# uthree/ALiVE-VC

Hardware: AMD Instinct MI355X
Metric: VC frames/sec + RTF @24kHz, 1M-vec library; 1/2/4/8 MI355X (higher is better)
Workload: dtype decoder fp16 GEMMs / fp32 acc; encoders 22-bit fp16 split; kNN exact fp32 top-k via fp6 MFMA candidates (certified); f32 MFMA small convs; f64 phase scan

## Files before the change

### alive-vc_amd/csrc/knn.hip

```cpp
#include "common.h"

namespace {

constexpr int D = ALIVE_DIM;
constexpr int KP = ALIVE_KPRIME;
constexpr int TILE = 128;
constexpr int MAX_SPLIT = 64;

__device__ __forceinline__ float wave_sum(float v) {
#pragma unroll
    for (int o = 32; o > 0; o >>= 1) v += __shfl_xor(v, o);
    return v;
}

struct NormDiv {
    float n, y;
};
__device__ __forceinline__ NormDiv norm_div(float n) {
    float y = __builtin_amdgcn_rcpf(n);
    const float e = fmaf(-n, y, 1.0f);
    y = fmaf(e, y, y);
    return NormDiv{n, y};
}
__device__ __forceinline__ float div_by(float x, const NormDiv& d) {
// ... 88 lines not shown
                                                                 const float* __restrict__ norms, int64_t M,
                                                                 unsigned* __restrict__ bound) {
    const int lane = threadIdx.x & 63;
    const int64_t m = (int64_t)blockIdx.x * 4 + (threadIdx.x >> 6);
    if (m >= M) return;
    const float nn = norms[m];
    float ss = 0.0f;
    for (int d = lane; d < D; d += 64) {
        const float q = rows[(size_t)m * D + d] / nn;
        const float b = __uint_as_float((unsigned)lib[(size_t)m * D + d] << 16);
        const float e = q - b;
        ss = fmaf(e, e, ss);
    }
    ss = wave_sum(ss);
    if (lane == 0) atomicMax(bound, __float_as_uint(sqrtf(ss) * 1.0001f));
}

constexpr float F8_SCALE = 256.0f;
constexpr float F6_SCALE = 32.0f;
__device__ __forceinline__ unsigned fp6_e2m3(float y) {
    const unsigned sgn = (__float_as_uint(y) >> 31) << 5;
    const float a = fminf(fabsf(y), 7.5f);
    unsigned code;
    if (a < 1.0f) {
        code = (unsigned)__builtin_rintf(a * 8.0f);
    } else {
        unsigned b = __float_as_uint(a);
        b += 0x7FFFFu + ((b >> 20) & 1u);
        code = (b >> 20) - (126u << 3);
        code = code < 31u ? code : 31u;
    }
    return sgn | code;
}
__global__ __launch_bounds__(256) void to_fp6_kernel(const unsigned short* __restrict__ in, int64_t n32, int64_t n_valid, u32x4* __restrict__ out,
                                                     unsigned char* __restrict__ clip = nullptr) {
    const int64_t i = (int64_t)blockIdx.x * 256 + threadIdx.x;
    if (i >= n32) return;
    if (i >= n_valid) {
        out[2 * i] = u32x4{0u, 0u, 0u, 0u};
        out[2 * i + 1] = u32x4{0u, 0u, 0u, 0u};
        return;
    }
    unsigned long long acc = 0;
    int nb = 0, wi = 0;
    unsigned wd[6];
    bool clipped = false;
#pragma unroll
    for (int j = 0; j < 32; ++j) {
        const float v = __uint_as_float((unsigned)in[i * 32 + j] << 16) * F6_SCALE;
        clipped = clipped || fabsf(v) > 7.75f;
        acc |= (unsigned long long)fp6_e2m3(v) << nb;
        nb += 6;
        if (nb >= 32) { wd[wi++] = (unsigned)acc; acc >>= 32; nb -= 32; }
    }
    out[2 * i] = u32x4{wd[0], wd[1], wd[2], wd[3]};
    out[2 * i + 1] = u32x4{wd[4], wd[5], 0u, 0u};
    if (clip != nullptr && clipped) clip[i / (D / 32)] = 1;
}
__device__ __forceinline__ unsigned char to_fp8(float v) {
    return (unsigned char)(__builtin_amdgcn_cvt_pk_fp8_f32(v * F8_SCALE, 0.0f, 0, false) & 0xff);
}
__device__ __forceinline__ unsigned to_fp8x4(float a, float b, float c, float d) {
    int w = __builtin_amdgcn_cvt_pk_fp8_f32(a * F8_SCALE, b * F8_SCALE, 0, false);
    w = __builtin_amdgcn_cvt_pk_fp8_f32(c * F8_SCALE, d * F8_SCALE, w, true);
    return (unsigned)w;
}

__global__ __launch_bounds__(256) void lib_to_fp8_kernel(const unsigned short* __restrict__ lib, int64_t n8, uint2* __restrict__ out) {
    const int64_t i = (int64_t)blockIdx.x * 256 + threadIdx.x;
    if (i >= n8) return;
    const u32x4 v = ((const u32x4*)lib)[i];
    float f[8];
#pragma unroll
    for (int j = 0; j < 4; ++j) {
        f[2 * j] = __uint_as_float(v[j] << 16);
        f[2 * j + 1] = __uint_as_float(v[j] & 0xffff0000u);
    }
    out[i] = make_uint2(to_fp8x4(f[0], f[1], f[2], f[3]), to_fp8x4(f[4], f[5], f[6], f[7]));
}

__global__ __launch_bounds__(256) void src_to_fp8_kernel(const unsigned short* __restrict__ s_bf16, int64_t n8, uint2* __restrict__ out) {
    const int64_t i = (int64_t)blockIdx.x * 256 + threadIdx.x;
    if (i >= n8) return;
    const u32x4 v = ((const u32x4*)s_bf16)[i];
    float f[8];
#pragma unroll
    for (int j = 0; j < 4; ++j) {
        f[2 * j] = __uint_as_float(v[j] << 16);
        f[2 * j + 1] = __uint_as_float(v[j] & 0xffff0000u);
    }
// ... 2173 lines not shown
    bool clipped = false;
#pragma unroll
    for (int h = 0; h < 2; ++h) {
#pragma unroll
        for (int j = 0; j < 32; ++j) {
            v[j] = live ? yb[(size_t)(32 * (cg + 8 * h) + j) * T] * inv : 0.0f;
            sy = fmaf(v[j], v[j], sy);
            v[j] *= F6_SCALE;
        }
        u32x4 o[2];
        clipped = fp6_slot(v, o) || clipped;
        if (f < Tt_pad) {
            u32x4* dst = (u32x4*)(out + (size_t)f * SUB_K + 32 * (cg + 8 * h));
            dst[0] = o[0];
            dst[1] = o[1];
        }
    }
    const float gy = live ? yb[(size_t)SUB_K * T] * inv : 0.0f;
    if (cg == 0) sy = fmaf(gy, gy, sy);
    ssq[cg][fl] = sy;
    clp[cg][fl] = clipped ? 1 : 0;
    __syncthreads();
    if (cg == 0 && f < Tt_pad) {
        float s2 = 0.0f;
        int cl = 0;
#pragma unroll
        for (int k = 0; k < 8; ++k) { s2 += ssq[k][fl]; cl |= clp[k][fl]; }
        const bool out_of_span = q > 0.0f && 1.0f - s2 > SUB_RES2;
        const bool bad = live && (cl != 0 || out_of_span);
        g[f] = gy;
        flag[f] = bad ? 1 : 0;
        if (bad) atomicAdd(stats + ST_SUB_FLAG, 1);
        if (live && cl != 0) atomicAdd(stats + ST_SUB_CLIP, 1);
    }
}
__global__ __launch_bounds__(256) void sub_select_kernel(const unsigned char* __restrict__ flag, unsigned char* __restrict__ clip6,
                                                         int64_t n, int* __restrict__ stats) {
    const bool sub = stats[ST_SUB_FLAG] <= RESEARCH_MIN;
    const int64_t i = (int64_t)blockIdx.x * 256 + threadIdx.x;
    if (sub && i < n && flag[i] != 0) clip6[i] = 1;
    if (i == 0) {
        stats[ST_SUB_FORM] = sub ? 1 : 2;
        stats[ST_SUB_GATE] = stats[ST_MODE] != 0 ? 0 : (sub ? 1 : 2);
    }
}

__global__ void stats_init_kernel(int* __restrict__ stats, int tier, int hist_tag = 0) {
    if (threadIdx.x < ST_HIST_TAG)
        stats[threadIdx.x] = threadIdx.x == ST_TIER ? tier
                           : threadIdx.x == ST_RESEARCH_MIN ? RESEARCH_MIN : threadIdx.x == ST_COLLECT_MIN ? COLLECT_MIN : 0;
    if (threadIdx.x == ST_HIST_TAG) {
        const bool valid = hist_tag != 0 && stats[ST_HIST_TAG] == hist_tag;
        const int streak = valid ? stats[ST_HIST_STREAK] : 0, calls = valid ? stats[ST_HIST_CALLS] : 0;
        const bool skip = streak >= PROBE_STREAK && (calls % PROBE_EVERY) != 0;
        stats[ST_HIST_TAG] = hist_tag;
        stats[ST_HIST_STREAK] = streak;
        stats[ST_HIST_CALLS] = calls + 1;
        stats[ST_PROBE_GATE] = skip ? 0 : 1;
        stats[ST_PROBE_SKIPPED] = skip ? 1 : 0;
    }
}
__global__ void probe_history_kernel(int* __restrict__ stats, int64_t Tt) {
    const bool clean = stats[ST_MODE] == 0 && (int64_t)stats[ST_FLAG8] * 20 <= Tt &&
                       (stats[ST_PROBE_GATE] == 0 || (int64_t)stats[ST_PROBE_FAIL] * 4 <= (int64_t)stats[ST_PROBE_N]);
    stats[ST_HIST_STREAK] = clean ? stats[ST_HIST_STREAK] + 1 : 0;
}
// ... 505 lines not shown
    if (g_ev_start) (void)hipEventRecord(g_ev_start, s);
    knn_scan_kernel<true><<<blocks, 64 * SCAN_WAVES, 0, s>>>(s_f32, rows_f32, norms, M, (int)Tt, k, pv, pi);
    if (g_ev_stop) (void)hipEventRecord(g_ev_stop, s);
    if (k <= 4) knn_scan_merge_kernel<true><<<(unsigned)Tt, 256, 0, s>>>(pv, pi, blocks * SCAN_WAVES, k, idx_base, out_val, out_idx);
    else knn_scan_merge_kernel<false><<<(unsigned)Tt, 256, 0, s>>>(pv, pi, blocks * SCAN_WAVES, k, idx_base, out_val, out_idx);
    ALIVE_CHECK_LAUNCH("alive_knn_search(scan)");
    return ALIVE_OK;
}

static void knn_exact_launch(const SearchWs& w, const float* rows_f32, const float* norms, int64_t M, int64_t Tt, int64_t idx_base,
                             int k, const int* list, const int* cnt, float* out_val, int32_t* out_idx, hipStream_t s,
                             int max_count = 0x7fffffff) {
#define ALIVE_EXACT(G_)                                                                                                        \
    {                                                                                                                          \
        knn_exact_kernel<G_><<<EX_BLOCKS, 256, 0, s>>>(w.s_f32, rows_f32, norms, M, Tt, k, list, cnt, w.pv, w.pi, max_count);   \
        knn_exact_merge_kernel<G_><<<1024, 256, 0, s>>>(w.pv, w.pi, Tt, k, idx_base, list, cnt, out_val, out_idx, max_count);  \
    }
    switch (exact_group(k)) {
        case 16: ALIVE_EXACT(16) break;
        case 8: ALIVE_EXACT(8) break;
        case 4: ALIVE_EXACT(4) break;
        case 2: ALIVE_EXACT(2) break;
        default: ALIVE_EXACT(1) break;
    }
#undef ALIVE_EXACT
}

static void src_prep_launch(const SearchWs& w, const float* src, int T, int64_t Tt, hipStream_t s) {
    float* dq = w.det_q != nullptr ? w.dq : nullptr;
    if (Tt <= 512) src_prep_small_kernel<<<(unsigned)w.p16.Tt_pad, 256, 0, s>>>(src, T, Tt, w.s_f32, w.s_bf16, dq, w.sub_nrm);
    else src_prep_kernel<<<(unsigned)(w.p16.Tt_pad / 64), 256, 0, s>>>(src, T, Tt, w.p16.Tt_pad, w.s_f32, w.s_bf16, dq, w.sub_nrm);
}

static int check_search_args(const char* what, const void* a, const void* b, int N, int T, int k, int64_t M) {
    ALIVE_CHECK_ARG(a && b, "%s: null pointer", what);
    ALIVE_CHECK_ARG(N > 0 && T > 0, "%s: empty source", what);
    ALIVE_CHECK_ARG(k >= 1 && k <= ALIVE_MAX_K, "%s: k=%d outside [1,%d]", what, k, ALIVE_MAX_K);
    ALIVE_CHECK_ARG(M >= k, "%s: library shard has %lld vectors, fewer than k=%d", what, (long long)M, k);
    ALIVE_CHECK_ARG((int64_t)N * T < ((int64_t)1 << 31) - FT6, "%s: %lld frames in one call", what, (long long)N * T);
    return ALIVE_OK;
}

static int lds_optin(const char* what) {
    static LdsOptIn optin8, optin6, optin16, optin_split, optin_sub;
    hipError_t e = optin8.ensure({(const void*)knn_score8_kernel, (const void*)knn_probe8_kernel}, SCORE8_LDS);
    if (e == hipSuccess) e = optin6.ensure({(const void*)knn_score6_kernel, (const void*)knn_probe6_kernel}, SCORE6_LDS);
    if (e == hipSuccess) e = optin16.ensure({(const void*)knn_score_kernel<false>, (const void*)knn_score_kernel<true>}, SCORE_LDS);
    if (e == hipSuccess) e = optin_split.ensure({(const void*)knn_collect_split_kernel}, SPLIT_LDS);
    if (e == hipSuccess) e = optin_sub.ensure({(const void*)knn_sub6_kernel}, SUB6_LDS);
    if (e != hipSuccess) {
        alive_set_error("%s: cannot reserve %d B of LDS: %s", what, SCORE_LDS, hipGetErrorString(e));
        return ALIVE_ERR_LAUNCH;
    }
    return ALIVE_OK;
}

extern "C" size_t alive_library_fp8_bytes(int64_t M) { return (size_t)alive_library_padded_rows(M) * D; }

extern "C" int alive_library_pack_fp8(const void* lib_bf16, int64_t M, void* lib_f8, void* stream) {
    ALIVE_CHECK_ARG(lib_bf16 && lib_f8 && M >= 1, "alive_library_pack_fp8: bad args");
    const int64_t n8 = alive_library_padded_rows(M) * D / 8;
    lib_to_fp8_kernel<<<(unsigned)((n8 + 255) / 256), 256, 0, (hipStream_t)stream>>>((const unsigned short*)lib_bf16, n8, (uint2*)lib_f8);
    ALIVE_CHECK_LAUNCH("alive_library_pack_fp8");
    return ALIVE_OK;
}

// ... 166 lines not shown
}

extern "C" int alive_knn_search_timed(const float* src, int N, int T, const void* lib_bf16, const float* rows_f32,
                                      const float* norms, int64_t M, int64_t idx_base, int k, float* out_val, int32_t* out_idx,
                                      void* ws, void* stream, void* ev_start, void* ev_stop) {
    return knn_search_impl(src, N, T, lib_bf16, rows_f32, norms, M, idx_base, k, out_val, out_idx, ws, stream,
                           (hipEvent_t)ev_start, (hipEvent_t)ev_stop);
}

static int knn_search_fp8_impl(const float* src, int N, int T, const void* lib_f8, const void* lib_bf16, const float* rows_f32,
                               const float* norms, int64_t M, int64_t idx_base, int k, float* out_val, int32_t* out_idx,
                               void* ws, void* stream, hipEvent_t g_ev_start, hipEvent_t g_ev_stop, int fmt = 0,
                               const float* y_rot = nullptr, float rot_c0 = 0.0f, const float* y_sub = nullptr,
                               const void* lib_sub = nullptr, const float* rho = nullptr) {
    ALIVE_CHECK_ARG(src && lib_f8 && lib_bf16 && rows_f32 && norms && out_val && out_idx && ws, "alive_knn_search_fp8: null pointer");
    if (int rc = check_search_args("alive_knn_search_fp8", src, ws, N, T, k, M)) return rc;
    const int64_t Tt = (int64_t)N * T;
    if (k > KH)
        return knn_search_impl(src, N, T, lib_bf16, rows_f32, norms, M, idx_base, k, out_val, out_idx, ws, stream, g_ev_start, g_ev_stop);
    const SearchWs w = ws_layout(ws, Tt, M, k, false, y_sub != nullptr);
    const bool f6 = fmt == 2;
    const SearchPlan& p = f6 ? w.p6 : w.p8;
    const SearchPlan& pp = f6 ? w.pp6 : w.pp;
    const int ft = f6 ? FT6 : FT, probe_pad = f6 ? w.probe_pad6 : w.probe_pad, lds = f6 ? SCORE6_LDS : SCORE8_LDS;
    const float pre = f6 ? 1.0f / (F6_SCALE * F6_SCALE) : 1.0f / (F8_SCALE * F8_SCALE),
                prior = f6 ? SD_PRIOR6 : (y_rot != nullptr ? SD_PRIOR8R : SD_PRIOR8);
    hipStream_t s = (hipStream_t)stream;
    if (Tt * k <= 64 && M <= SCAN_ROWS_MAX)
        return knn_scan_launch(src, T, Tt, rows_f32, norms, M, idx_base, k, w.s_f32, w.s_bf16, w.pv, w.pi, out_val, out_idx, w.stats, s, g_ev_start, g_ev_stop);
    if (int rc = lds_optin("alive_knn_search_fp8")) return rc;
    const int hist_tag = (int)(((uint64_t)M * 0x9E3779B1u) ^ ((uint64_t)Tt * 0x85EBCA77u) ^
                               (f6 ? (y_sub != nullptr ? 0x36u : 0x6u) : (y_rot != nullptr ? 0x18u : 0x8u))) | 1;
    stats_init_kernel<<<1, 64, 0, s>>>(w.stats, f6 ? TIER_FP6 : TIER_FP8, w.probe_n > 0 ? hist_tag : 0);
    src_prep_launch(w, src, T, Tt, s);
    if (f6) {
        const int64_t n32 = p.Tt_pad * D / 32;
        (void)hipMemsetAsync(w.clip6, 0, (size_t)p.Tt_pad, s);
        to_fp6_kernel<<<(unsigned)((n32 + 255) / 256), 256, 0, s>>>(w.s_bf16, n32, w.p16.Tt_pad * D / 32, (u32x4*)w.s_f8, w.clip6);
        if (y_sub != nullptr)
            sub_codes_kernel<<<(unsigned)(p.Tt_pad / 32), 256, 0, s>>>(y_sub, w.sub_nrm, T, Tt, p.Tt_pad, w.sub_f6, w.sub_g, w.sub_flag, w.stats);
    } else if (y_rot != nullptr) {
        rot_codes_kernel<<<(unsigned)(p.Tt_pad / 32), 256, 0, s>>>(y_rot, Tt, p.Tt_pad, T, 1, rot_c0, w.s_f8);
    } else {
        const int64_t n8 = p.Tt_pad * D / 8;
        src_to_fp8_kernel<<<(unsigned)((n8 + 255) / 256), 256, 0, s>>>(w.s_bf16, n8, (uint2*)w.s_f8);
    }
    int* mode = w.stats + ST_MODE;
    if (w.probe_n > 0) {
        const int* pgate = w.stats + ST_PROBE_GATE;
        probe_gather_kernel<<<(unsigned)probe_pad, 64, 0, s>>>(w.s_f8, Tt, w.probe_n, probe_pad, w.s_p8, w.p_list, pgate);
        if (f6)
            knn_probe6_kernel<<<dim3((unsigned)(probe_pad / ft), pp.split), 256, lds, s>>>(
                w.s_p8, (const unsigned char*)lib_f8, M, pp.tiles_total, pp.tiles_per_split, pp.P, w.cvp, w.cip, pgate);
        else
            knn_probe8_kernel<<<dim3((unsigned)(probe_pad / ft), pp.split), 256, lds, s>>>(
                w.s_p8, (const unsigned char*)lib_f8, M, pp.tiles_total, pp.tiles_per_split, pp.P, w.cvp, w.cip, pgate);
        rescore_launch((unsigned)((w.probe_n + 3) / 4), s, w.cvp, w.cip, pp.P, KP8, w.s_f32, rows_f32, norms, w.probe_n,
                                                                          idx_base, k, out_val, out_idx, w.p_list, pgate, GATE_BOOL, 0,
                                                                          w.p_list + probe_pad, w.stats + ST_PROBE_CNT, CERT_Z, KH8,
                                                                          pre, prior, nullptr, nullptr, nullptr, 0, 0.0f, f6 ? w.clip6 : nullptr);
        probe_decide_kernel<<<1, 1, 0, s>>>(w.stats, w.probe_n, PROBE_NUM, PROBE_DEN);
    }
    if (y_sub != nullptr) sub_select_kernel<<<(unsigned)((p.Tt_pad + 255) / 256), 256, 0, s>>>(w.sub_flag, w.clip6, p.Tt_pad, w.stats);
    const SeedArgs sa8 = seeds_for(w, p.Tt_pad / ft, p.split, k, f6 ? SEED_MARGIN6 : SEED_MARGIN8, ST_SEEDED, s, f6 ? SEED_MIN_FB6 : SEED_MIN_FB);
    if (g_ev_start) (void)hipEventRecord(g_ev_start, s);
    if (y_sub != nullptr) {
        const int* gate = w.stats + ST_SUB_GATE;
        knn_sub6_kernel<<<dim3((unsigned)(p.Tt_pad / ft), p.split), 256, SUB6_LDS, s>>>(
            w.sub_f6, (const unsigned char*)lib_sub, rho, w.sub_g, M, p.tiles_total, p.tiles_per_split, p.P, w.cv, w.ci, gate, 0, 1, sa8);
        knn_score6_kernel<<<dim3((unsigned)(p.Tt_pad / ft), p.split), 256, lds, s>>>(
            w.s_f8, (const unsigned char*)lib_f8, M, p.tiles_total, p.tiles_per_split, p.P, w.cv, w.ci, gate, 1, 2, sa8);
    } else if (f6)
        knn_score6_kernel<<<dim3((unsigned)(p.Tt_pad / ft), p.split), 256, lds, s>>>(
            w.s_f8, (const unsigned char*)lib_f8, M, p.tiles_total, p.tiles_per_split, p.P, w.cv, w.ci, mode, -1, 0, sa8);
    else
        knn_score8_kernel<<<dim3((unsigned)(p.Tt_pad / ft), p.split), 256, lds, s>>>(
            w.s_f8, (const unsigned char*)lib_f8, M, p.tiles_total, p.tiles_per_split, p.P, w.cv, w.ci, mode, -1, 0, sa8);
    if (g_ev_stop) (void)hipEventRecord(g_ev_stop, s);
    rescore_launch((unsigned)((Tt + 3) / 4), s, w.cv, w.ci, p.P, KP8, w.s_f32, rows_f32, norms, Tt, idx_base, k,
                                                               out_val, out_idx, nullptr, mode, -1, 0, w.list0, w.stats + ST_FLAG8,
                                                               CERT_Z, KH8, pre, prior, nullptr, nullptr, nullptr, 0, 0.0f, f6 ? w.clip6 : nullptr);
    if (w.probe_n > 0) flag_all_kernel<<<(unsigned)((Tt + 255) / 256), 256, 0, s>>>(w.list0, w.stats + ST_FLAG8, Tt, mode, 0, 1);
    if (w.probe_n > 0) probe_history_kernel<<<1, 1, 0, s>>>(w.stats, Tt);
    bf16_tiers_launch(w, lib_bf16, rows_f32, norms, M, Tt, idx_base, k, out_val, out_idx, s);
    ALIVE_CHECK_LAUNCH("alive_knn_search_fp8");
    return ALIVE_OK;
}

extern "C" int alive_knn_search_fp8(const float* src, int N, int T, const void* lib_f8, const void* lib_bf16, const float* rows_f32,
                                    const float* norms, int64_t M, int64_t idx_base, int k, float* out_val, int32_t* out_idx,
                                    void* ws, void* stream) {
    return knn_search_fp8_impl(src, N, T, lib_f8, lib_bf16, rows_f32, norms, M, idx_base, k, out_val, out_idx, ws, stream, nullptr, nullptr);
}
extern "C" int alive_knn_search_fp8_timed(const float* src, int N, int T, const void* lib_f8, const void* lib_bf16, const float* rows_f32,
                                          const float* norms, int64_t M, int64_t idx_base, int k, float* out_val, int32_t* out_idx,
                                          void* ws, void* stream, void* ev_start, void* ev_stop) {
// ... 11 lines not shown
    const int64_t span = m0 + count == M ? m_pad - m0 : count;
    ALIVE_CHECK_ARG(span % 32 == 0, "alive_library_pack_fp8_rot: a chunk that is not the last must hold a multiple of 32 rows");
    rot_codes_kernel<<<(unsigned)(span / 32), 256, 0, (hipStream_t)stream>>>(y_rows, count, span, 0, 0, c0, (unsigned char*)lib_f8 + (size_t)m0 * D);
    ALIVE_CHECK_LAUNCH("alive_library_pack_fp8_rot");
    return ALIVE_OK;
}
extern "C" int alive_knn_search_fp8_rot_timed(const float* src, const float* y_rot, float c0, int N, int T, const void* lib_f8_rot, const void* lib_bf16,
                                              const float* rows_f32, const float* norms, int64_t M, int64_t idx_base, int k, float* out_val,
                                              int32_t* out_idx, void* ws, void* stream, void* ev_start, void* ev_stop) {
    ALIVE_CHECK_ARG(y_rot != nullptr, "alive_knn_search_fp8_rot: null rotated frames");
    return knn_search_fp8_impl(src, N, T, lib_f8_rot, lib_bf16, rows_f32, norms, M, idx_base, k, out_val, out_idx, ws, stream,
                               (hipEvent_t)ev_start, (hipEvent_t)ev_stop, 0, y_rot, c0);
}

extern "C" int alive_knn_search_fp6(const float* src, int N, int T, const void* lib_f6, const void* lib_bf16, const float* rows_f32,
                                    const float* norms, int64_t M, int64_t idx_base, int k, float* out_val, int32_t* out_idx,
                                    void* ws, void* stream) {
    return knn_search_fp8_impl(src, N, T, lib_f6, lib_bf16, rows_f32, norms, M, idx_base, k, out_val, out_idx, ws, stream, nullptr, nullptr, 2);
}
extern "C" int alive_knn_search_fp6_timed(const float* src, int N, int T, const void* lib_f6, const void* lib_bf16, const float* rows_f32,
                                          const float* norms, int64_t M, int64_t idx_base, int k, float* out_val, int32_t* out_idx,
                                          void* ws, void* stream, void* ev_start, void* ev_stop) {
    return knn_search_fp8_impl(src, N, T, lib_f6, lib_bf16, rows_f32, norms, M, idx_base, k, out_val, out_idx, ws, stream,
                               (hipEvent_t)ev_start, (hipEvent_t)ev_stop, 2);
}

extern "C" int alive_knn_search_fp6_sub_timed(const float* src, const float* y_sub, int N, int T, const void* lib_sub, const float* rho,
                                              const void* lib_f6, const void* lib_bf16, const float* rows_f32, const float* norms, int64_t M,
                                              int64_t idx_base, int k, float* out_val, int32_t* out_idx, void* ws, void* stream,
                                              void* ev_start, void* ev_stop) {
    ALIVE_CHECK_ARG(y_sub && lib_sub && rho, "alive_knn_search_fp6_sub: null subspace operand");
    return knn_search_fp8_impl(src, N, T, lib_f6, lib_bf16, rows_f32, norms, M, idx_base, k, out_val, out_idx, ws, stream,
                               (hipEvent_t)ev_start, (hipEvent_t)ev_stop, 2, nullptr, 0.0f, y_sub, lib_sub, rho);
}
extern "C" int alive_knn_sub_coordinates(void) { return SUB_C; }
extern "C" size_t alive_library_fp6_sub_bytes(int64_t M) { return (size_t)alive_library_padded_rows(M) * SUB_K; }
extern "C" int alive_library_pack_fp6_sub(const float* y_rows, int64_t m0, int64_t count, int64_t M, void* lib_sub, float* rho, int* clip,
                                          void* stream) {
    ALIVE_CHECK_ARG(y_rows && lib_sub && rho && clip && M >= 1 && m0 >= 0 && count >= 1 && m0 + count <= M && (m0 % 32) == 0,
                    "alive_library_pack_fp6_sub: bad args (m0 must be a multiple of 32)");
    const int64_t m_pad = alive_library_padded_rows(M);
    const int64_t span = m0 + count == M ? m_pad - m0 : count;
    const int64_t n = span * (SUB_K / 32);
    lib_sub6_kernel<<<(unsigned)((n + 255) / 256), 256, 0, (hipStream_t)stream>>>(y_rows, count, span, (unsigned char*)lib_sub + (size_t)m0 * SUB_K,
                                                                                 rho + m0, clip);
    ALIVE_CHECK_LAUNCH("alive_library_pack_fp6_sub");
    return ALIVE_OK;
}

extern "C" const int* alive_knn_search_stats(int N, int T, int64_t M, void* ws) {
    return ws_layout(ws, (int64_t)N * T, M, 4).stats;
}

extern "C" int alive_knn_merge_gather(const float* cand_val, const int32_t* cand_idx, int n_shards, int k, double alpha,
                                      const float* rows_f32_full, const float* src, int N, int T, float* out,
                                      int32_t* final_idx, void* stream) {
    ALIVE_CHECK_ARG(cand_val && cand_idx && rows_f32_full && src && out, "alive_knn_merge_gather: null pointer");
    ALIVE_CHECK_ARG(k >= 1 && k <= ALIVE_MAX_K && n_shards >= 1 && n_shards * k <= 512,
                    "alive_knn_merge_gather: n_shards*k = %d exceeds 512", n_shards * k);
    ALIVE_CHECK_ARG(N > 0 && T > 0, "alive_knn_merge_gather: empty source");
    const int zs = (int64_t)cdiv(T, 32) * N < 64 ? D / 64 : 1;
    const dim3 g(cdiv(T, 32), N, zs);
    if (k <= 8 && n_shards * k <= 128)
        knn_merge_gather_kernel<2, 8><<<g, 256, 0, (hipStream_t)stream>>>(cand_val, cand_idx, n_shards, k, (float)alpha,
                                                                       (float)(1.0 - alpha), rows_f32_full, src, T, (int64_t)N * T, out, final_idx);
    else
// ... 282 lines not shown
```

### alive-vc_amd/module/_native.py

```python
import ctypes as C
import os

import torch

_HERE = os.path.dirname(os.path.abspath(__file__))
LIB_PATH = os.environ.get("ALIVE_VC_LIB", os.path.join(os.path.dirname(_HERE), "libalive_vc.so"))

_lib = None


class AliveConv(C.Structure):
    _fields_ = [
        ("W", C.c_void_p), ("bias", C.c_void_p), ("X", C.c_void_p),
        ("N", C.c_int), ("Ci", C.c_int), ("Tin", C.c_int), ("Co", C.c_int), ("K_pad", C.c_int),
        ("KW", C.c_int), ("stride", C.c_int), ("dil", C.c_int), ("pad_left", C.c_int), ("pad_mode", C.c_int),
        ("Tout", C.c_int), ("up", C.c_int), ("act", C.c_int),
        ("post_add", C.c_void_p), ("ch_scale", C.c_void_p), ("residual", C.c_void_p), ("skip", C.c_void_p),
        ("Y", C.c_void_p), ("Z", C.c_void_p), ("film", C.c_void_p),
        ("film_rows", C.c_int), ("Lf", C.c_int), ("film_scale_row", C.c_int), ("film_shift_row", C.c_int),
        ("precision", C.c_int), ("Ci_pad", C.c_int),
        ("film_t0", C.c_int), ("film_f0", C.c_int), ("film_ld", C.c_int),
        ("Xp", C.c_void_p), ("Zp", C.c_void_p), ("Yp", C.c_void_p), ("yp_planes", C.c_int),
    ]

# ... 7 lines not shown
        ("b_plane", C.c_int64), ("b_win", C.c_int64), ("b_row", C.c_int), ("b_cblk", C.c_int), ("b_blk", C.c_int64),
        ("arg_val", C.c_void_p), ("arg_idx", C.c_void_p),
        ("Y2", C.c_void_p), ("y_split", C.c_int),
        ("f16s", C.c_int), ("wscale", C.c_void_p), ("in_unscale", C.c_float), ("pout_scale", C.c_float),
    ]


_VP, _I, _I64, _F, _D, _SZ = C.c_void_p, C.c_int, C.c_int64, C.c_float, C.c_double, C.c_size_t

PROTOTYPES = {
    "alive_last_error": (C.c_char_p, []),
    "alive_version": (_I, []),
    "alive_library_padded_rows": (_I64, [_I64]),
    "alive_library_pack": (_I, [_VP, _I64, _I, _VP, _VP, _VP, _VP]),
    "alive_knn_workspace_bytes": (_SZ, [_I64, _I64]),
    "alive_knn_workspace_bytes_strict": (_SZ, [_I64, _I64]),
    "alive_knn_workspace_bytes_fast": (_SZ, [_I64, _I64]),
    "alive_knn_search": (_I, [_VP, _I, _I, _VP, _VP, _VP, _I64, _I64, _I, _VP, _VP, _VP, _VP]),
    "alive_library_fp8_bytes": (_SZ, [_I64]),
    "alive_library_rounding_bound": (_I, [_VP, _VP, _VP, _I64, _VP, _VP]),
    "alive_library_pack_lo": (_I, [_VP, _VP, _VP, _I64, _VP, _VP]),
    "alive_knn_search_strict": (_I, [_VP, _I, _I, _VP, _VP, _VP, _VP, _VP, _I64, _I64, _I, _VP, _VP, _VP, _VP, _VP, _VP]),
    "alive_library_pack_fp8": (_I, [_VP, _I64, _VP, _VP]),
    "alive_knn_search_fp8": (_I, [_VP, _I, _I, _VP, _VP, _VP, _VP, _I64, _I64, _I, _VP, _VP, _VP, _VP]),
    "alive_knn_search_stats": (_VP, [_I, _I, _I64, _VP]),
    "alive_knn_search_timed": (_I, [_VP, _I, _I, _VP, _VP, _VP, _I64, _I64, _I, _VP, _VP, _VP, _VP, _VP, _VP]),
    "alive_knn_search_fp8_timed": (_I, [_VP, _I, _I, _VP, _VP, _VP, _VP, _I64, _I64, _I, _VP, _VP, _VP, _VP, _VP, _VP]),
    "alive_library_pack_fp6": (_I, [_VP, _I64, _VP, _VP]),
    "alive_knn_sub_coordinates": (_I, []),
    "alive_knn_workspace_bytes_sub": (_SZ, [_I64, _I64]),
    "alive_library_fp6_sub_bytes": (_SZ, [_I64]),
    "alive_library_pack_fp6_sub": (_I, [_VP, _I64, _I64, _I64, _VP, _VP, _VP, _VP]),
    "alive_knn_search_fp6_sub_timed": (_I, [_VP, _VP, _I, _I, _VP, _VP, _VP, _VP, _VP, _VP, _I64, _I64, _I, _VP, _VP, _VP, _VP, _VP, _VP]),
    "alive_knn_rot_coordinates": (_I, []),
    "alive_knn_rot_leading": (_I, []),
    "alive_knn_rot_mixed": (_I, []),
    "alive_library_pack_fp8_rot": (_I, [_VP, _I64, _I64, _I64, _F, _VP, _VP]),
    "alive_knn_search_fp8_rot_timed": (_I, [_VP, _VP, _F, _I, _I, _VP, _VP, _VP, _VP, _I64, _I64, _I, _VP, _VP, _VP, _VP, _VP, _VP]),
    "alive_knn_search_fp6": (_I, [_VP, _I, _I, _VP, _VP, _VP, _VP, _I64, _I64, _I, _VP, _VP, _VP, _VP]),
    "alive_knn_search_fp6_timed": (_I, [_VP, _I, _I, _VP, _VP, _VP, _VP, _I64, _I64, _I, _VP, _VP, _VP, _VP, _VP, _VP]),
    "alive_library_pack_rows": (_I, [_VP, _I64, _I, _VP, _VP, _VP]),
    "alive_knn_grouped_workspace_bytes": (_SZ, [_I, _I, _I]),
    "alive_knn_search_grouped": (_I, [_VP, _I, _I, _VP, _VP, _I64, _VP, _VP, _I, _VP, _VP, _VP, _VP]),
    "alive_knn_merge_gather_rows": (_I, [_VP, _VP, _I, _VP, _VP, _VP, _I, _I, _VP, _VP, _VP]),
    "alive_knn_blend_gather_rows": (_I, [_VP, _VP, _I, _VP, _VP, _VP, _VP, _VP, _I, _I, _VP, _VP]),
    "alive_pool_append": (_I, [_VP, _I64, _I64, _I64, _I, _VP, _VP, _I64, _I64, _VP, _VP]),
    "alive_pool_move_rows": (_I, [_VP, _VP, _I64, _I64, _I64, _I64, _VP]),
    "alive_pool_image_bytes": (_SZ, [_VP, _I, _VP]),
    "alive_pool_pack_images": (_I, [_VP, _VP, _I64, _VP, _VP, _I, _VP, _VP, _VP]),
    "alive_knn_pool_workspace_bytes": (_SZ, [_I, _I, _I, _I, _I64, _I64]),
    "alive_knn_search_pool": (_I, [_VP, _I, _I, _VP, _VP, _VP, _VP, _VP, _I64, _VP, _VP, _I, _I64, _VP, _I, _VP, _VP, _VP, _VP]),
    "alive_knn_pool_stats": (_VP, [_VP]),
    "alive_dedup_pass": (_I, [_VP, _VP, _I64, _I, _D, _VP, _VP, _VP]),
    "alive_knn_merge_gather": (_I, [_VP, _VP, _I, _I, _D, _VP, _VP, _I, _I, _VP, _VP, _VP]),
    "alive_conv1d": (_I, [C.POINTER(AliveConv), _VP]),
    "alive_decoder_precision": (_I, [_I]),
    "alive_encoder_precision": (_I, [_I]),
    "alive_f16_saturations": (_I, [_I]),
    "alive_f16_saturations_clear": (_I, [_VP]),
    "alive_gelu_film": (_I, [_VP, _I, _I, _I, _VP, _I, _I, _I, _I, _I, _I, _I, _VP, _VP, _VP]),
    "alive_planes_bytes": (_SZ, [_I64, _I, _I]),
    "alive_to_planes": (_I, [_VP, _I, _I, _I, _I, _VP, _VP]),
    "alive_gemm_planes": (_I, [C.POINTER(AliveGemm), _VP]),
    "alive_argmax_merge": (_I, [_VP, _VP, _I, _I64, _VP, _VP]),
    "alive_filter_block_small_weights": (_I, [_I]),
    "alive_filter_block_small": (_I, [_VP, _I, _I, _I, _VP, _VP, _I, _I, _I, _VP, _VP, _VP]),
# ... 129 lines not shown
```

### include/alive_vc.h

```cpp
#ifndef ALIVE_VC_H
#define ALIVE_VC_H

#include <stddef.h>
#include <stdint.h>

#ifdef __cplusplus
extern "C" {
#endif

#define ALIVE_OK 0
#define ALIVE_ERR_ARG (-1)
#define ALIVE_ERR_LAUNCH (-2)

#define ALIVE_DIM 768
#define ALIVE_KPRIME 16
#define ALIVE_MAX_K 64

const char* alive_last_error(void);
int alive_version(void);

int64_t alive_library_padded_rows(int64_t M);
int alive_library_pack(const float* tokens_DxM, int64_t M, int D,
                       void* lib_bf16, float* rows_f32, float* norms, void* stream);

// ... 28 lines not shown
int alive_knn_search_fp8_timed(const float* src, int N, int T,
                               const void* lib_f8, const void* lib_bf16, const float* rows_f32, const float* norms,
                               int64_t M, int64_t idx_base, int k,
                               float* out_val, int32_t* out_idx, void* ws, void* stream, void* ev_start, void* ev_stop);

int alive_knn_rot_coordinates(void);
int alive_knn_rot_leading(void);
int alive_knn_rot_mixed(void);
int alive_library_pack_fp8_rot(const float* y_rows, int64_t m0, int64_t count, int64_t M, float c0, void* lib_f8, void* stream);
int alive_knn_search_fp8_rot_timed(const float* src, const float* y_rot, float c0, int N, int T,
                                   const void* lib_f8_rot, const void* lib_bf16, const float* rows_f32, const float* norms,
                                   int64_t M, int64_t idx_base, int k,
                                   float* out_val, int32_t* out_idx, void* ws, void* stream, void* ev_start, void* ev_stop);

int alive_library_pack_fp6(const void* lib_bf16, int64_t M, void* lib_f6, void* stream);
int alive_knn_search_fp6(const float* src, int N, int T,
                         const void* lib_f6, const void* lib_bf16, const float* rows_f32, const float* norms,
                         int64_t M, int64_t idx_base, int k,
                         float* out_val, int32_t* out_idx, void* ws, void* stream);
int alive_knn_search_fp6_timed(const float* src, int N, int T,
                               const void* lib_f6, const void* lib_bf16, const float* rows_f32, const float* norms,
                               int64_t M, int64_t idx_base, int k,
                               float* out_val, int32_t* out_idx, void* ws, void* stream, void* ev_start, void* ev_stop);

int alive_knn_sub_coordinates(void);
size_t alive_knn_workspace_bytes_sub(int64_t Tt, int64_t M);
size_t alive_library_fp6_sub_bytes(int64_t M);
int alive_library_pack_fp6_sub(const float* y_rows, int64_t m0, int64_t count, int64_t M, void* lib_sub, float* rho, int* clip,
                               void* stream);
int alive_knn_search_fp6_sub_timed(const float* src, const float* y_sub, int N, int T, const void* lib_sub, const float* rho,
                                   const void* lib_f6, const void* lib_bf16, const float* rows_f32, const float* norms, int64_t M,
                                   int64_t idx_base, int k, float* out_val, int32_t* out_idx, void* ws, void* stream,
                                   void* ev_start, void* ev_stop);

int alive_knn_merge_gather(const float* cand_val, const int32_t* cand_idx, int n_shards, int k,
                           double alpha, const float* rows_f32_full, const float* src,
                           int N, int T, float* out, int32_t* final_idx, void* stream);

int alive_library_pack_rows(const float* tokens, int64_t M, int Dd, float* rows_f32, float* norms, void* stream);
size_t alive_knn_grouped_workspace_bytes(int N, int T, int k);
int alive_knn_search_grouped(const float* src, int N, int T, const float* rows_f32, const float* norms, int64_t P,
                             const int32_t* seg_lo, const int32_t* seg_len, int k, float* out_val, int32_t* out_idx,
                             void* ws, void* stream);
int alive_knn_merge_gather_rows(const float* cand_val, const int32_t* cand_idx, int k, const double* alpha,
                                const float* rows_f32_full, const float* src, int N, int T, float* out,
                                int32_t* final_idx, void* stream);
#define ALIVE_MAX_BLEND 4
int alive_knn_blend_gather_rows(const float* cand_val, const int32_t* cand_idx, int k, const int32_t* first,
                                const double* weight, const double* alpha, const float* rows_f32_full, const float* src,
                                int N, int T, float* out, void* stream);

int alive_pool_append(const float* tokens, int64_t row_stride, int64_t col_stride, int64_t M, int Dd, float* rows_f32,
                      float* norms, int64_t capacity, int64_t at, int32_t* report, void* stream);
int alive_pool_move_rows(float* rows_f32, float* norms, int64_t capacity, int64_t src, int64_t dst, int64_t n, void* stream);

#define ALIVE_POOL_STATS 8
size_t alive_pool_image_bytes(const int32_t* seg_len, int V, int64_t* img_off);
int alive_pool_pack_images(const float* rows_f32, const float* norms, int64_t P, const int32_t* seg_lo, const int32_t* seg_len,
                           int V, void* images, float* bounds, void* stream);
size_t alive_knn_pool_workspace_bytes(int N, int T, int k, int V, int64_t P, int64_t max_len);
int alive_knn_search_pool(const float* src, int N, int T, const void* images, const int64_t* img_off, const float* rows_f32,
                          const float* norms, const float* bounds, int64_t P, const int32_t* seg_lo, const int32_t* seg_len,
                          int V, int64_t max_len, const int32_t* voice, int k, float* out_val, int32_t* out_idx, void* ws,
                          void* stream);
const int* alive_knn_pool_stats(void* ws);

// ... 194 lines not shown
```

Baseline: 1.343 million.

## Fuse subspace source prep and code generation; gate full fp6 conversion on subspace outcome

```diff
diff --git a/alive-vc_amd/csrc/knn.hip b/alive-vc_amd/csrc/knn.hip
--- a/alive-vc_amd/csrc/knn.hip
+++ b/alive-vc_amd/csrc/knn.hip
@@ -144,10 +144,8 @@
     }
     return sgn | code;
 }
-__global__ __launch_bounds__(256) void to_fp6_kernel(const unsigned short* __restrict__ in, int64_t n32, int64_t n_valid, u32x4* __restrict__ out,
-                                                     unsigned char* __restrict__ clip = nullptr) {
-    const int64_t i = (int64_t)blockIdx.x * 256 + threadIdx.x;
-    if (i >= n32) return;
+__device__ __forceinline__ void to_fp6_group(const unsigned short* __restrict__ in, int64_t i, int64_t n_valid, u32x4* __restrict__ out,
+                                             unsigned char* __restrict__ clip) {
     if (i >= n_valid) {
         out[2 * i] = u32x4{0u, 0u, 0u, 0u};
         out[2 * i + 1] = u32x4{0u, 0u, 0u, 0u};
@@ -168,6 +166,28 @@
     out[2 * i] = u32x4{wd[0], wd[1], wd[2], wd[3]};
     out[2 * i + 1] = u32x4{wd[4], wd[5], 0u, 0u};
     if (clip != nullptr && clipped) clip[i / (D / 32)] = 1;
+}
+__global__ __launch_bounds__(256) void to_fp6_kernel(const unsigned short* __restrict__ in, int64_t n32, int64_t n_valid, u32x4* __restrict__ out,
+                                                     unsigned char* __restrict__ clip = nullptr) {
+    const int64_t i = (int64_t)blockIdx.x * 256 + threadIdx.x;
+    if (i >= n32) return;
+    to_fp6_group(in, i, n_valid, out, clip);
+}
+__global__ __launch_bounds__(256) void to_fp6_gated_kernel(const unsigned short* __restrict__ in, int64_t n32, int64_t n_valid,
+                                                           u32x4* __restrict__ out, unsigned char* __restrict__ clip,
+                                                           const int* __restrict__ gate, int want) {
+    if (*gate != want) return;
+    const int64_t i = (int64_t)blockIdx.x * 256 + threadIdx.x;
+    if (i >= n32) return;
+    to_fp6_group(in, i, n_valid, out, clip);
+}
+__global__ __launch_bounds__(256) void to_fp6_sample_kernel(const unsigned short* __restrict__ in, int64_t Tt, int n, u32x4* __restrict__ out,
+                                                            unsigned char* __restrict__ clip, const int* __restrict__ gate) {
+    if (*gate == 0) return;
+    const int i = blockIdx.x * 256 + threadIdx.x;
+    if (i >= n * (D / 32)) return;
+    const int64_t ft = (int64_t)(i / (D / 32)) * Tt / n;
+    to_fp6_group(in, ft * (D / 32) + i % (D / 32), Tt * (D / 32), out, clip);
 }
 __device__ __forceinline__ unsigned char to_fp8(float v) {
     return (unsigned char)(__builtin_amdgcn_cvt_pk_fp8_f32(v * F8_SCALE, 0.0f, 0, false) & 0xff);
@@ -2407,6 +2427,108 @@
         flag[f] = bad ? 1 : 0;
         if (bad) atomicAdd(stats + ST_SUB_FLAG, 1);
         if (live && cl != 0) atomicAdd(stats + ST_SUB_CLIP, 1);
+    }
+}
+__global__ __launch_bounds__(512, 4) void sub_prep_kernel(const float* __restrict__ src, const float* __restrict__ y, int T, int64_t Tt,
+                                                          int64_t Tp16, int64_t Tp6, float* __restrict__ s_f32,
+                                                          unsigned short* __restrict__ s_bf16, float* __restrict__ nrm_out,
+                                                          unsigned char* __restrict__ out, float* __restrict__ g,
+                                                          unsigned char* __restrict__ flag, int* __restrict__ stats) {
+    __shared__ float red[4][64];
+    __shared__ float tile[2][64][65];
+    __shared__ float nrm[64];
+    __shared__ float ssq[8][64];
+    __shared__ int clp[8][64];
+    constexpr int H = D / 8;
+    const int lane = threadIdx.x & 63, wv = threadIdx.x >> 6, w4 = wv & 3, half = wv >> 2;
+    const int64_t f0 = (int64_t)blockIdx.x * 64;
+    const int64_t ft = f0 + lane;
+    const bool ok = ft < Tt;
+    const int64_t n = ok ? ft / T : 0;
+    const int t = ok ? (int)(ft - n * T) : 0;
+    const float* col = src + (size_t)n * D * T + t;
+    float x[H];
+#pragma unroll
+    for (int m = 0; m < H; ++m) x[m] = ok ? col[(size_t)(w4 + 4 * (H * half + m)) * T] : 0.0f;
+    if (half == 0) {
+        float ss = 0.0f;
+#pragma unroll
+        for (int m = 0; m < H; ++m) ss = fmaf(x[m], x[m], ss);
+        red[w4][lane] = ss;
+    }
+    __syncthreads();
+    if (half == 1) {
+        float ss = red[w4][lane];
+#pragma unroll
+        for (int m = 0; m < H; ++m) ss = fmaf(x[m], x[m], ss);
+        red[w4][lane] = ss;
+    }
+    __syncthreads();
+    if (wv == 0) {
+        nrm[lane] = sqrtf(red[0][lane] + red[1][lane] + red[2][lane] + red[3][lane]);
+        if (ok) nrm_out[ft] = nrm[lane];
+    }
+    __syncthreads();
+#pragma unroll
+    for (int c = 0; c < H / 16; ++c) {
+        const int d0 = 64 * (c + (H / 16) * half);
+#pragma unroll
+        for (int i = 0; i < 16; ++i) tile[half][w4 + 4 * i][lane] = x[16 * c + i];
+        __syncthreads();
+#pragma unroll 4
+        for (int i = 0; i < 16; ++i) {
+            const int r = w4 + 4 * i;
+            const int64_t ff = f0 + r;
+            if (ff < Tp16) {
+                const float q = (ff < Tt && nrm[r] > 0.0f) ? tile[half][lane][r] / nrm[r] : 0.0f;
+                if (ff < Tt) s_f32[(size_t)ff * D + d0 + lane] = q;
+                s_bf16[(size_t)ff * D + d0 + lane] = f32_to_bf16_rn(q);
+            }
+        }
+        __syncthreads();
+    }
+    const float* yb = y + (size_t)n * SUB_C * T + t;
+    const float q = ok ? nrm[lane] : 0.0f;
+    const float inv = q > 0.0f ? 1.0f / q : 0.0f;
+    const int cg = wv;
+    float v[32];
+    float sy = 0.0f;
+    bool clipped = false;
+#pragma unroll 1
+    for (int h = 0; h < 2; ++h) {
+#pragma unroll
+        for (int j = 0; j < 32; ++j) {
+            v[j] = ok ? yb[(size_t)(32 * (cg + 8 * h) + j) * T] * inv : 0.0f;
+            sy = fmaf(v[j], v[j], sy);
+            v[j] *= F6_SCALE;
+        }
+        u32x4 o[2];
+        clipped = fp6_slot(v, o) || clipped;
+        if (ft < Tp6) {
+            u32x4* dst = (u32x4*)(out + (size_t)ft * SUB_K + 32 * (cg + 8 * h));
+            dst[0] = o[0];
+            dst[1] = o[1];
+        }
+    }
+    float gy = 0.0f;
+    if (cg == 0) {
+        gy = ok ? yb[(size_t)SUB_K * T] * inv : 0.0f;
+        sy = fmaf(gy, gy, sy);
+    }
+    ssq[cg][lane] = sy;
+    clp[cg][lane] = clipped ? 1 : 0;
+    __syncthreads();
+    if (wv == 0 && ft < Tp6) {
+        float s2 = 0.0f;
+        int cl = 0;
+#pragma unroll
+        for (int k = 0; k < 8; ++k) { s2 += ssq[k][lane]; cl |= clp[k][lane]; }
+        const bool out_of_span = q > 0.0f && 1.0f - s2 > SUB_RES2;
+        const bool bad = ok && (cl != 0 || out_of_span);
+        g[ft] = gy;
+        flag[ft] = bad ? 1 : 0;
+        if (bad) atomicAdd(stats + ST_SUB_FLAG, 1);
+        if (ok && cl != 0) atomicAdd(stats + ST_SUB_CLIP, 1);
     }
 }
 __global__ __launch_bounds__(256) void sub_select_kernel(const unsigned char* __restrict__ flag, unsigned char* __restrict__ clip6,
@@ -2978,6 +3100,17 @@
     else src_prep_kernel<<<(unsigned)(w.p16.Tt_pad / 64), 256, 0, s>>>(src, T, Tt, w.p16.Tt_pad, w.s_f32, w.s_bf16, dq, w.sub_nrm);
 }
 
+static void sub_prep_launch(const SearchWs& w, const float* src, const float* y_sub, int T, int64_t Tt, hipStream_t s, bool fused) {
+    const int64_t Tp6 = w.p6.Tt_pad, Tp16 = w.p16.Tt_pad;
+    if (fused && Tt > 512 && w.det_q == nullptr) {
+        sub_prep_kernel<<<(unsigned)((Tp6 > Tp16 ? Tp6 : Tp16) / 64), 512, 0, s>>>(src, y_sub, T, Tt, Tp16, Tp6, w.s_f32, w.s_bf16, w.sub_nrm,
+                                                                                   w.sub_f6, w.sub_g, w.sub_flag, w.stats);
+        return;
+    }
+    src_prep_launch(w, src, T, Tt, s);
+    sub_codes_kernel<<<(unsigned)(Tp6 / 32), 256, 0, s>>>(y_sub, w.sub_nrm, T, Tt, Tp6, w.sub_f6, w.sub_g, w.sub_flag, w.stats);
+}
+
 static int check_search_args(const char* what, const void* a, const void* b, int N, int T, int k, int64_t M) {
     ALIVE_CHECK_ARG(a && b, "%s: null pointer", what);
     ALIVE_CHECK_ARG(N > 0 && T > 0, "%s: empty source", what);
@@ -3210,22 +3343,27 @@
     const int hist_tag = (int)(((uint64_t)M * 0x9E3779B1u) ^ ((uint64_t)Tt * 0x85EBCA77u) ^
                                (f6 ? (y_sub != nullptr ? 0x36u : 0x6u) : (y_rot != nullptr ? 0x18u : 0x8u))) | 1;
     stats_init_kernel<<<1, 64, 0, s>>>(w.stats, f6 ? TIER_FP6 : TIER_FP8, w.probe_n > 0 ? hist_tag : 0);
-    src_prep_launch(w, src, T, Tt, s);
-    if (f6) {
-        const int64_t n32 = p.Tt_pad * D / 32;
+    const int64_t n32 = p.Tt_pad * D / 32;
+    if (y_sub != nullptr) {
+        sub_prep_launch(w, src, y_sub, T, Tt, s, true);
+        (void)hipMemsetAsync(w.clip6, 0, (size_t)p.Tt_pad, s);
+    } else if (f6) {
+        src_prep_launch(w, src, T, Tt, s);
         (void)hipMemsetAsync(w.clip6, 0, (size_t)p.Tt_pad, s);
         to_fp6_kernel<<<(unsigned)((n32 + 255) / 256), 256, 0, s>>>(w.s_bf16, n32, w.p16.Tt_pad * D / 32, (u32x4*)w.s_f8, w.clip6);
-        if (y_sub != nullptr)
-            sub_codes_kernel<<<(unsigned)(p.Tt_pad / 32), 256, 0, s>>>(y_sub, w.sub_nrm, T, Tt, p.Tt_pad, w.sub_f6, w.sub_g, w.sub_flag, w.stats);
     } else if (y_rot != nullptr) {
+        src_prep_launch(w, src, T, Tt, s);
         rot_codes_kernel<<<(unsigned)(p.Tt_pad / 32), 256, 0, s>>>(y_rot, Tt, p.Tt_pad, T, 1, rot_c0, w.s_f8);
     } else {
+        src_prep_launch(w, src, T, Tt, s);
         const int64_t n8 = p.Tt_pad * D / 8;
         src_to_fp8_kernel<<<(unsigned)((n8 + 255) / 256), 256, 0, s>>>(w.s_bf16, n8, (uint2*)w.s_f8);
     }
     int* mode = w.stats + ST_MODE;
     if (w.probe_n > 0) {
         const int* pgate = w.stats + ST_PROBE_GATE;
+        if (y_sub != nullptr)
+            to_fp6_sample_kernel<<<(unsigned)((w.probe_n * (D / 32) + 255) / 256), 256, 0, s>>>(w.s_bf16, Tt, w.probe_n, (u32x4*)w.s_f8, w.clip6, pgate);
         probe_gather_kernel<<<(unsigned)probe_pad, 64, 0, s>>>(w.s_f8, Tt, w.probe_n, probe_pad, w.s_p8, w.p_list, pgate);
         if (f6)
             knn_probe6_kernel<<<dim3((unsigned)(probe_pad / ft), pp.split), 256, lds, s>>>(
@@ -3239,7 +3377,11 @@
                                                                           pre, prior, nullptr, nullptr, nullptr, 0, 0.0f, f6 ? w.clip6 : nullptr);
         probe_decide_kernel<<<1, 1, 0, s>>>(w.stats, w.probe_n, PROBE_NUM, PROBE_DEN);
     }
-    if (y_sub != nullptr) sub_select_kernel<<<(unsigned)((p.Tt_pad + 255) / 256), 256, 0, s>>>(w.sub_flag, w.clip6, p.Tt_pad, w.stats);
+    if (y_sub != nullptr) {
+        sub_select_kernel<<<(unsigned)((p.Tt_pad + 255) / 256), 256, 0, s>>>(w.sub_flag, w.clip6, p.Tt_pad, w.stats);
+        to_fp6_gated_kernel<<<(unsigned)((n32 + 255) / 256), 256, 0, s>>>(w.s_bf16, n32, w.p16.Tt_pad * D / 32, (u32x4*)w.s_f8, w.clip6,
+                                                                         w.stats + ST_SUB_GATE, 2);
+    }
     const SeedArgs sa8 = seeds_for(w, p.Tt_pad / ft, p.split, k, f6 ? SEED_MARGIN6 : SEED_MARGIN8, ST_SEEDED, s, f6 ? SEED_MIN_FB6 : SEED_MIN_FB);
     if (g_ev_start) (void)hipEventRecord(g_ev_start, s);
     if (y_sub != nullptr) {
@@ -3317,6 +3459,25 @@
     ALIVE_CHECK_ARG(y_sub && lib_sub && rho, "alive_knn_search_fp6_sub: null subspace operand");
     return knn_search_fp8_impl(src, N, T, lib_f6, lib_bf16, rows_f32, norms, M, idx_base, k, out_val, out_idx, ws, stream,
                                (hipEvent_t)ev_start, (hipEvent_t)ev_stop, 2, nullptr, 0.0f, y_sub, lib_sub, rho);
+}
+extern "C" int alive_knn_sub_frame_prep(const float* src, const float* y_sub, int N, int T, int64_t M, void* ws, int fused, void* stream) {
+    ALIVE_CHECK_ARG(src && y_sub && ws && N > 0 && T > 0 && M >= 1, "alive_knn_sub_frame_prep: bad args");
+    const int64_t Tt = (int64_t)N * T;
+    const SearchWs w = ws_layout(ws, Tt, M, 4, false, true);
+    stats_init_kernel<<<1, 64, 0, (hipStream_t)stream>>>(w.stats, TIER_FP6);
+    sub_prep_launch(w, src, y_sub, T, Tt, (hipStream_t)stream, fused != 0);
+    ALIVE_CHECK_LAUNCH("alive_knn_sub_frame_prep");
+    return ALIVE_OK;
+}
+extern "C" const void* alive_knn_sub_operand(int which, int N, int T, int64_t M, void* ws, size_t* bytes) {
+    const int64_t Tt = (int64_t)N * T;
+    const SearchWs w = ws_layout(ws, Tt, M, 4, false, true);
+    const size_t Tp16 = (size_t)w.p16.Tt_pad, Tp6 = (size_t)w.p6.Tt_pad;
+    const void* ptr[6] = {w.s_f32, w.s_bf16, w.sub_nrm, w.sub_f6, w.sub_g, w.sub_flag};
+    const size_t len[6] = {(size_t)Tt * D * 4, Tp16 * D * 2, (size_t)Tt * 4, Tp6 * SUB_K, Tp6 * 4, Tp6};
+    if (which < 0 || which > 5) return nullptr;
+    if (bytes != nullptr) *bytes = len[which];
+    return ptr[which];
 }
 extern "C" int alive_knn_sub_coordinates(void) { return SUB_C; }
 extern "C" size_t alive_library_fp6_sub_bytes(int64_t M) { return (size_t)alive_library_padded_rows(M) * SUB_K; }
diff --git a/alive-vc_amd/module/_native.py b/alive-vc_amd/module/_native.py
--- a/alive-vc_amd/module/_native.py
+++ b/alive-vc_amd/module/_native.py
@@ -63,6 +63,8 @@
     "alive_library_fp6_sub_bytes": (_SZ, [_I64]),
     "alive_library_pack_fp6_sub": (_I, [_VP, _I64, _I64, _I64, _VP, _VP, _VP, _VP]),
     "alive_knn_search_fp6_sub_timed": (_I, [_VP, _VP, _I, _I, _VP, _VP, _VP, _VP, _VP, _VP, _I64, _I64, _I, _VP, _VP, _VP, _VP, _VP, _VP]),
+    "alive_knn_sub_frame_prep": (_I, [_VP, _VP, _I, _I, _I64, _VP, _I, _VP]),
+    "alive_knn_sub_operand": (_VP, [_I, _I, _I, _I64, _VP, _VP]),
     "alive_knn_rot_coordinates": (_I, []),
     "alive_knn_rot_leading": (_I, []),
     "alive_knn_rot_mixed": (_I, []),
diff --git a/include/alive_vc.h b/include/alive_vc.h
--- a/include/alive_vc.h
+++ b/include/alive_vc.h
@@ -84,6 +84,8 @@
                                    const void* lib_f6, const void* lib_bf16, const float* rows_f32, const float* norms, int64_t M,
                                    int64_t idx_base, int k, float* out_val, int32_t* out_idx, void* ws, void* stream,
                                    void* ev_start, void* ev_stop);
+int alive_knn_sub_frame_prep(const float* src, const float* y_sub, int N, int T, int64_t M, void* ws, int fused, void* stream);
+const void* alive_knn_sub_operand(int which, int N, int T, int64_t M, void* ws, size_t* bytes);
 
 int alive_knn_merge_gather(const float* cand_val, const int32_t* cand_idx, int n_shards, int k,
                            double alpha, const float* rows_f32_full, const float* src,
```

New measurement: 1.345 million, median of 4. No clear change (+0.2%).
